# GabeTsai/YOLO-For-Turbines

Measured on AMD Instinct MI355X. Metric: images/sec at 416x416 (fwd), higher is better.
Workload: dtype f32; 1 GPU; BASELINE configs[1]: batch 32/GPU 416x416 fp32 inference, 80-class head, YOLOv3 forward (75 fused conv launches); per_gpu_batch=32, global_batch=32, image_size=416, num_classes=80, parallelism=image-sharded x1 (no collective)

## Files before the change

yolo_for_turbines_amd/csrc/conv_split3_f32.hip:

```cpp
#include "conv_f32_epilogue.h"
#include "split3.h"

namespace yolo {

constexpr int S3_ROWB = 64;

__device__ __forceinline__ int s3_row_off(int r, int chunk) { return r * S3_ROWB + (((chunk >> 1) ^ ((r >> 2) & 3)) * 16 + (chunk & 1) * 8); }

typedef const __attribute__((address_space(1))) void* s3_gptr;
typedef __attribute__((address_space(3))) void* s3_lptr;
__device__ __forceinline__ void s3_glds16(const void* g, void* l) { __builtin_amdgcn_global_load_lds((s3_gptr)g, (s3_lptr)l, 16, 0, 0); }

struct S3PrepArgs {
    const float* w;
    char* out;
    int Kpad, KT, cp;
};

__global__ __launch_bounds__(256) void split3_weights_f32(const S3PrepArgs p) {
    const int tid = threadIdx.x;
    const int chunk = tid & 7;
    const int n = blockIdx.x * 32 + (tid >> 3);
    const size_t plane_b = (size_t)p.cp * S3_ROWB;
    const float* src = p.w + (size_t)n * p.Kpad + chunk * 4;
    char* dst = p.out + s3_row_off(n, chunk);
    f32x4 chk = {0.f, 0.f, 0.f, 0.f};
    for (int kt = 0; kt < p.KT; ++kt) {
        const f32x4 v = *reinterpret_cast<const f32x4*>(src + kt * BK);
        u32x2 h, m, l;
        s3_split(v, h, m, l, chk);
        char* d = dst + (size_t)kt * 3 * plane_b;
        *reinterpret_cast<u32x2*>(d) = h;
        *reinterpret_cast<u32x2*>(d + plane_b) = m;
        *reinterpret_cast<u32x2*>(d + 2 * plane_b) = l;
    }
    const bool nonfinite = chk[0] != chk[0] || chk[1] != chk[1] || chk[2] != chk[2] || chk[3] != chk[3];
    const int any = __syncthreads_or(nonfinite);
    if (tid == 0) reinterpret_cast<unsigned*>(p.out + (size_t)p.KT * 3 * plane_b)[blockIdx.x] = any ? 1u : 0u;
}

template <int BM, int BN, bool WREADY, bool WDMA>
__global__ __launch_bounds__(256, 2) void conv_split3_f32(const ConvArgs p) {
    static_assert(WREADY || !WDMA, "LDS-DMA needs the prepared weights");
    constexpr int WM = BM / 2, WN = BN / 2;
    constexpr int TM = WM / 32, TN = WN / 32;
    constexpr int RA = BM / 32, RB = BN / 32;
    constexpr bool DBUF = BM + BN <= 128;
    constexpr int A_BYTES = 3 * BM * S3_ROWB;
    constexpr int B_BYTES = 3 * BN * S3_ROWB;
    constexpr int BUF_BYTES = A_BYTES + B_BYTES;
    constexpr bool BRING = DBUF || WDMA;
    constexpr int B_SLOT = DBUF ? BUF_BYTES : B_BYTES;
    constexpr int PB = BN / 64;
    extern __shared__ __attribute__((aligned(16))) char smem_raw[];

    const int tid = threadIdx.x;
    const int lane = tid & 63;
    const int wave = tid >> 6;
    const int wm = wave >> 1, wn = wave & 1;
    const int tile_n = blockIdx.x % p.tiles_n;
    const int tile_m = blockIdx.x / p.tiles_n;
    const int m0 = tile_m * BM, n0 = tile_n * BN;
    const int HoWo = p.Ho * p.Wo;

    auto row_geom = [&](int m, long long& base, unsigned& mask) {
        const bool mv = m < p.M;
        const int mm = mv ? m : 0;
        const int n = mm / HoWo;
        const int rem = mm - n * HoWo;
        const int ho = rem / p.Wo;
        const int wo = rem - ho * p.Wo;
        const int hi0 = ho * p.stride - p.pad, wi0 = wo * p.stride - p.pad;
        base = ((long long)(n * p.H + hi0) * p.W + wi0) * p.x_ld + p.x_off;
        unsigned mk = 0;
        for (int kh = 0; kh < p.ks; ++kh)
            for (int kw = 0; kw < p.ks; ++kw)
                if (mv && (unsigned)(hi0 + kh) < (unsigned)p.H && (unsigned)(wi0 + kw) < (unsigned)p.W)
                    mk |= 1u << (kh * p.ks + kw);
        mask = mk;
    };

    const int chunk = tid & 7;
    const int lrow = tid >> 3;
    long long a_base[RA];
    unsigned a_mask[RA];
#pragma unroll
    for (int i = 0; i < RA; ++i) row_geom(m0 + lrow + 32 * i, a_base[i], a_mask[i]);
    const float* wrow = p.w + (size_t)(n0 + lrow) * p.Kpad + chunk * 4;
    const char* wq = p.w_planes;
    const size_t plane_b = (size_t)((p.Cout + 127) & ~127) * S3_ROWB;
    const char* wsrc = wq + (size_t)n0 * S3_ROWB + tid * 16;

    f32x4 ra[RA], rb[RB];
    s3_u32x4 rw[3][PB];
    f32x4 chk = {0.f, 0.f, 0.f, 0.f};
    auto load_global = [&](int kt) {
        const int kg = kt * BK;
        const int tap = kg / p.Cin;
        const int coff = kg - tap * p.Cin + chunk * 4;
        const int kh = tap / p.ks, kw = tap - kh * p.ks;
        const long long toff = (long long)(kh * p.W + kw) * p.x_ld + coff;
#pragma unroll
        for (int i = 0; i < RA; ++i) {
            const bool v = (a_mask[i] >> tap) & 1u;
            f32x4 z = {0.f, 0.f, 0.f, 0.f};
            ra[i] = v ? *reinterpret_cast<const f32x4*>(p.x + a_base[i] + toff) : z;
        }
        if constexpr (!WREADY) {
#pragma unroll
            for (int i = 0; i < RB; ++i)
                rb[i] = *reinterpret_cast<const f32x4*>(wrow + (size_t)(32 * i) * p.Kpad + kt * BK);
        } else {
            const char* src = wsrc + (size_t)kt * 3 * plane_b;
            char* dst = smem_raw + A_BYTES + (kt & 1) * B_SLOT + wave * 1024;
#pragma unroll
            for (int q = 0; q < 3; ++q)
#pragma unroll
                for (int i = 0; i < PB; ++i) {
                    if constexpr (WDMA)
                        s3_glds16(src + q * plane_b + i * 4096, dst + q * BN * S3_ROWB + i * 4096);
                    else
                        rw[q][i] = *reinterpret_cast<const s3_u32x4*>(src + q * plane_b + i * 4096);
                }
        }
    };
    auto store_lds = [&](int buf, int bslot) {
        char* a = smem_raw + buf * BUF_BYTES + s3_row_off(lrow, chunk);
        char* b = smem_raw + A_BYTES + bslot * B_SLOT + s3_row_off(lrow, chunk);
#pragma unroll
        for (int i = 0; i < RA; ++i) {
            u32x2 h, m, l;
            s3_split(ra[i], h, m, l, chk);
            *reinterpret_cast<u32x2*>(a + (0 * BM + 32 * i) * S3_ROWB) = h;
            *reinterpret_cast<u32x2*>(a + (1 * BM + 32 * i) * S3_ROWB) = m;
            *reinterpret_cast<u32x2*>(a + (2 * BM + 32 * i) * S3_ROWB) = l;
        }
        if constexpr (!WREADY) {
#pragma unroll
            for (int i = 0; i < RB; ++i) {
                u32x2 h, m, l;
                s3_split(rb[i], h, m, l, chk);
                *reinterpret_cast<u32x2*>(b + (0 * BN + 32 * i) * S3_ROWB) = h;
                *reinterpret_cast<u32x2*>(b + (1 * BN + 32 * i) * S3_ROWB) = m;
                *reinterpret_cast<u32x2*>(b + (2 * BN + 32 * i) * S3_ROWB) = l;
            }
        } else if constexpr (!WDMA) {
            char* bw = smem_raw + A_BYTES + bslot * B_SLOT + tid * 16;
#pragma unroll
            for (int q = 0; q < 3; ++q)
#pragma unroll
                for (int i = 0; i < PB; ++i) *reinterpret_cast<s3_u32x4*>(bw + q * BN * S3_ROWB + i * 4096) = rw[q][i];
        }
    };

    f32x16 acc[TM][TN];
#pragma unroll
    for (int i = 0; i < TM; ++i)
#pragma unroll
        for (int j = 0; j < TN; ++j)
#pragma unroll
            for (int r = 0; r < 16; ++r) acc[i][j][r] = 0.f;

    const int frow = lane & 31, fh = lane >> 5;
    const int a_frag = (wm * WM + frow) * S3_ROWB;
    const int b_frag = A_BYTES + (wn * WN + frow) * S3_ROWB;
    const int fsw = (frow >> 2) & 3;
    const int f_slot[2] = {(fh ^ fsw) * 16, ((2 + fh) ^ fsw) * 16};

    load_global(0);
    store_lds(0, 0);
    if constexpr (WDMA) asm volatile("s_waitcnt vmcnt(0)" ::: "memory");
    __syncthreads();

    for (int kt = 0; kt < p.KT; ++kt) {
        const int cur = DBUF ? (kt & 1) : 0;
        const int bcur = BRING ? (kt & 1) : 0;
        const bool more = kt + 1 < p.KT;
        if (more) load_global(kt + 1);
        const char* Ab = smem_raw + cur * BUF_BYTES + a_frag;
        const char* Bb = smem_raw + bcur * B_SLOT + b_frag;
#pragma unroll
        for (int c = 0; c < 2; ++c) {
            s3_bf16x8 af[TM][3], bf[TN][3];
#pragma unroll
            for (int i = 0; i < TM; ++i)
#pragma unroll
                for (int q = 0; q < 3; ++q)
                    af[i][q] = *reinterpret_cast<const s3_bf16x8*>(Ab + (q * BM + i * 32) * S3_ROWB + f_slot[c]);
#pragma unroll
            for (int j = 0; j < TN; ++j)
#pragma unroll
                for (int q = 0; q < 3; ++q)
                    bf[j][q] = *reinterpret_cast<const s3_bf16x8*>(Bb + (q * BN + j * 32) * S3_ROWB + f_slot[c]);
            constexpr int QA[6] = {0, 2, 1, 0, 1, 0};
            constexpr int QB[6] = {2, 0, 1, 1, 0, 0};
#pragma unroll
            for (int t = 0; t < 6; ++t)
#pragma unroll
                for (int i = 0; i < TM; ++i)
#pragma unroll
                    for (int j = 0; j < TN; ++j)
                        acc[i][j] = __builtin_amdgcn_mfma_f32_32x32x16_bf16(af[i][QA[t]], bf[j][QB[t]], acc[i][j], 0, 0, 0);
        }
        if (!DBUF) __syncthreads();
        if (more) store_lds(DBUF ? (cur ^ 1) : 0, BRING ? (bcur ^ 1) : 0);
        if constexpr (WDMA) asm volatile("s_waitcnt vmcnt(0)" ::: "memory");
        __syncthreads();
    }

    bool nonfinite = chk[0] != chk[0] || chk[1] != chk[1] || chk[2] != chk[2] || chk[3] != chk[3];
    if constexpr (WREADY) {
        const unsigned* table = reinterpret_cast<const unsigned*>(wq + (size_t)p.KT * 3 * plane_b);
#pragma unroll
        for (int g = 0; g < BN / 32; ++g) nonfinite |= table[n0 / 32 + g] != 0;
    }
    if (__syncthreads_or(nonfinite)) {
        long long f_base[TM];
        unsigned f_mask[TM];
#pragma unroll
        for (int i = 0; i < TM; ++i) row_geom(m0 + wm * WM + i * 32 + frow, f_base[i], f_mask[i]);
        const float* fw = p.w + (size_t)(n0 + wn * WN + frow) * p.Kpad + 4 * fh;
#pragma unroll
        for (int i = 0; i < TM; ++i)
#pragma unroll
            for (int j = 0; j < TN; ++j)
#pragma unroll
                for (int r = 0; r < 16; ++r) acc[i][j][r] = 0.f;
        for (int kt = 0; kt < p.KT; ++kt) {
            const int kg = kt * BK;
            const int tap = kg / p.Cin;
            const int kh = tap / p.ks, kw = tap - kh * p.ks;
            const long long toff = (long long)(kh * p.W + kw) * p.x_ld + (kg - tap * p.Cin) + 4 * fh;
            for (int s = 0; s < 4; ++s) {
                f32x4 af[TM], bf[TN];
#pragma unroll
                for (int i = 0; i < TM; ++i) {
                    f32x4 z = {0.f, 0.f, 0.f, 0.f};
                    af[i] = ((f_mask[i] >> tap) & 1u) ? *reinterpret_cast<const f32x4*>(p.x + f_base[i] + toff + s * 8) : z;
                }
#pragma unroll
                for (int j = 0; j < TN; ++j) bf[j] = *reinterpret_cast<const f32x4*>(fw + (size_t)(32 * j) * p.Kpad + kg + s * 8);
#pragma unroll
                for (int e = 0; e < 4; ++e)
#pragma unroll
                    for (int i = 0; i < TM; ++i)
#pragma unroll
                        for (int j = 0; j < TN; ++j)
                            acc[i][j] = __builtin_amdgcn_mfma_f32_32x32x2f32(af[i][e], bf[j][e], acc[i][j], 0, 0, 0);
            }
        }
    }

    conv_f32_epilogue<BM, BN>(p, acc, reinterpret_cast<float*>(smem_raw), m0, n0);
}

bool split3_supported(const yolo_conv_desc* d) {
    return d->dtype == YOLO_F32 && (d->ksize == 1 || d->ksize == 3) && (d->stride == 1 || d->stride == 2) && d->cin % 32 == 0;
}

template <int BM, int BN, bool WREADY, bool WDMA>
static int launch_split3(const ConvArgs& a, hipStream_t s) {
    constexpr bool dbuf = BM + BN <= 128;
    constexpr size_t operands = dbuf ? (size_t)2 * 3 * (BM + BN) * S3_ROWB : (size_t)3 * (BM + (WDMA ? 2 : 1) * BN) * S3_ROWB;
    constexpr size_t transpose = (size_t)BM * (BN + 4) * sizeof(float);
    constexpr size_t lds = operands > transpose ? operands : transpose;
    ConvArgs p = a;
    p.tiles_n = ceil_div(a.Cout, BN);
    const long long blocks = (long long)ceil_div(a.M, BM) * p.tiles_n;
    if (blocks > 0x7fffffffLL) return fail(YOLO_ERR_UNSUPPORTED, "conv_split3_f32: too many blocks");
    if (lds > 64 * 1024) {
        static LdsOnce once;
        if (int rc = reserve_lds(once, reinterpret_cast<const void*>(&conv_split3_f32<BM, BN, WREADY, WDMA>), lds, "conv_split3_f32")) return rc;
    }
    hipLaunchKernelGGL((conv_split3_f32<BM, BN, WREADY, WDMA>), dim3((unsigned)blocks), dim3(256), lds, s, p);
    return check_launch("conv_split3_f32");
}

constexpr bool kS3Dma128x128 = true, kS3Dma128x64 = false, kS3Dma64x64 = true;

template <int BM, int BN, bool WDMA>
static int launch_split3(const ConvArgs& a, hipStream_t s) {
    return a.w_planes ? launch_split3<BM, BN, true, WDMA>(a, s) : launch_split3<BM, BN, false, false>(a, s);
}

size_t split3_weight_bytes(const yolo_conv_desc* d) {
    const size_t cp = coutpad_of(d->cout), KT = kpad_of(d->cin, d->ksize) / BK;
    return packed_f32(d->cout, d->cin, d->ksize).tail_bytes + KT * 3 * cp * S3_ROWB + cp / 32 * sizeof(unsigned);
}

int split3_weights_launch(const yolo_conv_desc* d, const void* w_packed, void* out, hipStream_t s) {
    const size_t off = packed_f32(d->cout, d->cin, d->ksize).tail_bytes;
    if (out != w_packed) {
        const char *a = static_cast<const char*>(w_packed), *b = static_cast<const char*>(out);
        if (a < b + split3_weight_bytes(d) && b < a + off) return fail(YOLO_ERR_ARG, "yolo_split3_weights: out overlaps w_packed (pass the same pointer to prepare in place)");
        if (hipMemcpyAsync(out, w_packed, off, hipMemcpyDeviceToDevice, s) != hipSuccess) return check_launch("yolo_split3_weights: copy");
    }
    S3PrepArgs p;
    p.w = static_cast<const float*>(w_packed);
    p.out = static_cast<char*>(out) + off;
    p.Kpad = kpad_of(d->cin, d->ksize);
    p.KT = p.Kpad / BK;
    p.cp = coutpad_of(d->cout);
    hipLaunchKernelGGL(split3_weights_f32, dim3(p.cp / 32), dim3(256), 0, s, p);
    return check_launch("split3_weights_f32");
}

static int pick_split3_tile(const ConvArgs& a, bool ready) {
    if (a.ks == 3 && a.stride == 2 && a.Cin >= 64 && (ready || a.Cin < 512)) return kTileF32Reg128x128;
    if (a.ks == 1 && (long long)a.H * a.W * a.Cout < 100000) return kTileF32Reg64x64;
    if (ready && a.ks == 1 && a.Cout % 128 == 0 && a.Cin >= ((long long)a.H * a.W >= 52 * 52 ? 256 : 768)) return kTileF32Reg128x128;
    return kTileF32Reg128x64;
}

bool split3_eligible(const yolo_conv_desc* d) {
    if (!split3_supported(d)) return false;
    if (d->ksize == 3) return d->stride == 2 || (d->cin == 32 && (long long)d->h * d->w >= 208 * 208);
    return d->stride == 1 && (long long)d->h * d->w * d->cout >= 40000;
}

int conv_split3_launch(const ConvArgs& a, int tile, hipStream_t s) {
    switch (tile ? tile : pick_split3_tile(a, a.w_planes != nullptr)) {
    case kTileF32Reg128x128: return launch_split3<128, 128, kS3Dma128x128>(a, s);
    case kTileF32Reg128x64: return launch_split3<128, 64, kS3Dma128x64>(a, s);
    case kTileF32Reg64x64: return launch_split3<64, 64, kS3Dma64x64>(a, s);
    default: return fail(YOLO_ERR_UNSUPPORTED, "conv: YOLO_FLAG_SPLIT_BF16 has tiles 1 (128x128), 2 (128x64) and 4 (64x64), not %d", tile);
    }
}

}
```

Baseline: 3223 images/s.

## Peel last k-step, use scalar-addressed weight DMA and branchless A loads

Splits the conv main loop into a templated step with a peeled final iteration, so the prefetch condition becomes compile-time. Weight DMA now uses a wave-uniform scalar base with per-lane offsets through a shared helper. A-tile loads always read, falling back to a padding address when the tap is out of bounds, and zero the data at split time. Adds sched_barriers around the MFMA block, and the barrier waits only on lgkmcnt in the DMA path. The aim is to cut per-lane address math and branch divergence and to give better load/compute scheduling, at the risk of extra loads from the padding address and reliance on p.x_off.

```diff
diff --git a/yolo_for_turbines_amd/csrc/conv_split3_f32.hip b/yolo_for_turbines_amd/csrc/conv_split3_f32.hip
--- a/yolo_for_turbines_amd/csrc/conv_split3_f32.hip
+++ b/yolo_for_turbines_amd/csrc/conv_split3_f32.hip
@@ -1,15 +1,20 @@
 #include "conv_f32_epilogue.h"
 #include "split3.h"
+#include "wino_dma.h"
 
 namespace yolo {
 
+template <bool WDMA>
+__device__ __forceinline__ void s3_sync() {
+    if constexpr (WDMA) asm volatile("s_waitcnt lgkmcnt(0)\n\ts_barrier" ::: "memory");
+    else __syncthreads();
+}
+
 constexpr int S3_ROWB = 64;
 
 __device__ __forceinline__ int s3_row_off(int r, int chunk) { return r * S3_ROWB + (((chunk >> 1) ^ ((r >> 2) & 3)) * 16 + (chunk & 1) * 8); }
 
-typedef const __attribute__((address_space(1))) void* s3_gptr;
 typedef __attribute__((address_space(3))) void* s3_lptr;
-__device__ __forceinline__ void s3_glds16(const void* g, void* l) { __builtin_amdgcn_global_load_lds((s3_gptr)g, (s3_lptr)l, 16, 0, 0); }
 
 struct S3PrepArgs {
     const float* w;
@@ -90,35 +95,44 @@
     const char* wq = p.w_planes;
     const size_t plane_b = (size_t)((p.Cout + 127) & ~127) * S3_ROWB;
     const char* wsrc = wq + (size_t)n0 * S3_ROWB + tid * 16;
+    const int wave_u = __builtin_amdgcn_readfirstlane(wave);
+    const char* wdma_src = wq + (size_t)n0 * S3_ROWB + wave_u * 1024;
+    const unsigned wdma_dst = (unsigned)(size_t)(s3_lptr)smem_raw + A_BYTES + wave_u * 1024;
 
     f32x4 ra[RA], rb[RB];
+    unsigned av;
     s3_u32x4 rw[3][PB];
     f32x4 chk = {0.f, 0.f, 0.f, 0.f};
-    auto load_global = [&](int kt) {
+    auto load_a = [&](int kt) {
         const int kg = kt * BK;
         const int tap = kg / p.Cin;
         const int coff = kg - tap * p.Cin + chunk * 4;
         const int kh = tap / p.ks, kw = tap - kh * p.ks;
         const long long toff = (long long)(kh * p.W + kw) * p.x_ld + coff;
+        unsigned valid = 0;
 #pragma unroll
         for (int i = 0; i < RA; ++i) {
             const bool v = (a_mask[i] >> tap) & 1u;
-            f32x4 z = {0.f, 0.f, 0.f, 0.f};
-            ra[i] = v ? *reinterpret_cast<const f32x4*>(p.x + a_base[i] + toff) : z;
-        }
+            valid |= (unsigned)v << i;
+            ra[i] = *reinterpret_cast<const f32x4*>(p.x + (v ? a_base[i] + toff : (long long)p.x_off + coff));
+        }
+        av = valid;
+    };
+    auto load_b = [&](int kt) {
         if constexpr (!WREADY) {
 #pragma unroll
             for (int i = 0; i < RB; ++i)
                 rb[i] = *reinterpret_cast<const f32x4*>(wrow + (size_t)(32 * i) * p.Kpad + kt * BK);
         } else {
             const char* src = wsrc + (size_t)kt * 3 * plane_b;
-            char* dst = smem_raw + A_BYTES + (kt & 1) * B_SLOT + wave * 1024;
+            const char* dsrc = wdma_src + (size_t)kt * 3 * plane_b;
+            const unsigned dst = wdma_dst + (kt & 1) * B_SLOT;
 #pragma unroll
             for (int q = 0; q < 3; ++q)
 #pragma unroll
                 for (int i = 0; i < PB; ++i) {
                     if constexpr (WDMA)
-                        s3_glds16(src + q * plane_b + i * 4096, dst + q * BN * S3_ROWB + i * 4096);
+                        wn_glds16_s(dsrc + q * plane_b + i * 4096, lane * 16, dst + q * BN * S3_ROWB + i * 4096);
                     else
                         rw[q][i] = *reinterpret_cast<const s3_u32x4*>(src + q * plane_b + i * 4096);
                 }
@@ -130,7 +144,8 @@
 #pragma unroll
         for (int i = 0; i < RA; ++i) {
             u32x2 h, m, l;
-            s3_split(ra[i], h, m, l, chk);
+            const f32x4 z = {0.f, 0.f, 0.f, 0.f};
+            s3_split((av >> i) & 1u ? ra[i] : z, h, m, l, chk);
             *reinterpret_cast<u32x2*>(a + (0 * BM + 32 * i) * S3_ROWB) = h;
             *reinterpret_cast<u32x2*>(a + (1 * BM + 32 * i) * S3_ROWB) = m;
             *reinterpret_cast<u32x2*>(a + (2 * BM + 32 * i) * S3_ROWB) = l;
@@ -167,16 +182,15 @@
     const int fsw = (frow >> 2) & 3;
     const int f_slot[2] = {(fh ^ fsw) * 16, ((2 + fh) ^ fsw) * 16};
 
-    load_global(0);
-    store_lds(0, 0);
-    if constexpr (WDMA) asm volatile("s_waitcnt vmcnt(0)" ::: "memory");
-    __syncthreads();
-
-    for (int kt = 0; kt < p.KT; ++kt) {
+    auto step = [&](auto MORE, int kt) {
+        constexpr bool more = decltype(MORE)::value;
         const int cur = DBUF ? (kt & 1) : 0;
         const int bcur = BRING ? (kt & 1) : 0;
-        const bool more = kt + 1 < p.KT;
-        if (more) load_global(kt + 1);
+        if constexpr (more) {
+            load_b(kt + 1);
+            load_a(kt + 1);
+        }
+        __builtin_amdgcn_sched_barrier(0);
         const char* Ab = smem_raw + cur * BUF_BYTES + a_frag;
         const char* Bb = smem_raw + bcur * B_SLOT + b_frag;
 #pragma unroll
@@ -202,11 +216,21 @@
                     for (int j = 0; j < TN; ++j)
                         acc[i][j] = __builtin_amdgcn_mfma_f32_32x32x16_bf16(af[i][QA[t]], bf[j][QB[t]], acc[i][j], 0, 0, 0);
         }
-        if (!DBUF) __syncthreads();
-        if (more) store_lds(DBUF ? (cur ^ 1) : 0, BRING ? (bcur ^ 1) : 0);
-        if constexpr (WDMA) asm volatile("s_waitcnt vmcnt(0)" ::: "memory");
-        __syncthreads();
-    }
+        __builtin_amdgcn_sched_barrier(0);
+        if (!DBUF) s3_sync<WDMA>();
+        if constexpr (more) store_lds(DBUF ? (cur ^ 1) : 0, BRING ? (bcur ^ 1) : 0);
+        if constexpr (WDMA) wn_wait_vmcnt<0>();
+        s3_sync<WDMA>();
+    };
+
+    load_b(0);
+    load_a(0);
+    store_lds(0, 0);
+    if constexpr (WDMA) wn_wait_vmcnt<0>();
+    s3_sync<WDMA>();
+
+    for (int kt = 0; kt + 1 < p.KT; ++kt) step(std::true_type{}, kt);
+    step(std::false_type{}, p.KT - 1);
 
     bool nonfinite = chk[0] != chk[0] || chk[1] != chk[1] || chk[2] != chk[2] || chk[3] != chk[3];
     if constexpr (WREADY) {
```

New measurement: 3271 images/s (median of 6 runs). 1.02x the previous value.
